# alexkreimer/libviso

Hardware: AMD Instinct MI355X
Metric: stereo_frames_per_sec_1241x376_matcher (higher is better)
Workload: dtype u16; 1 GPU; configs[1]: synthetic 1241x376 stereo pairs, 2000 features/image, SAD matcher only (pack + 3 match_desc/frame + sort)

## Files before the change

libviso_amd/csrc/match_union8.hip:

```cpp
#include "common.h"
#include "match_dev.h"
#include <stddef.h>
#include <stdlib.h>

#define MU_THREADS 256
#define MU_WAVES 4
#define MU_QPB 64
#define MU_G 8
#define MU_UCAP 448
#define MU_PAD 32
#ifndef MU_NP
#define MU_NP 2
#endif
#ifndef MU_RNP
#define MU_RNP 2
#endif
#define MU_S8ROWS 176
#define MU_KPCAP 512
#define MU_NBY 64

template <int CTRL>
__device__ __forceinline__ uint32_t mu_dpp(uint32_t v) {
    return (uint32_t)__builtin_amdgcn_update_dpp(0, (int)v, CTRL, 0xf, 0xf, false);
}

template <int CTRL>
__device__ __forceinline__ uint32_t mu_bcast(uint32_t v) {
    return (uint32_t)__builtin_amdgcn_update_dpp(0, (int)v, CTRL, 0xf, 0xf, true);
}

__device__ __forceinline__ float mu_fmin(float a, float b) { float r; asm("v_min_f32_e32 %0, %1, %2" : "=v"(r) : "v"(a), "v"(b)); return r; }
__device__ __forceinline__ float mu_fmax(float a, float b) { float r; asm("v_max_f32_e32 %0, %1, %2" : "=v"(r) : "v"(a), "v"(b)); return r; }

__device__ __forceinline__ uint32_t mu_l1_bits(float qx, float qy, float2 t) {
    const float dx = qx - t.x, dy = qy - t.y;
    float d;
    asm("v_add_f32_e64 %0, |%1|, |%2|" : "=v"(d) : "v"(dx), "v"(dy));
    return __float_as_uint(d);
}

struct MuTrack { uint32_t m1, m2, m3; };

__device__ __forceinline__ uint32_t mu_med3(uint32_t a, uint32_t b, uint32_t c) {
    uint32_t r;
    asm("v_med3_u32 %0, %1, %2, %3" : "=v"(r) : "v"(a), "v"(b), "v"(c));
    return r;
}

__device__ __forceinline__ void mu_update(MuTrack& t, uint32_t key) {
    t.m3 = mu_med3(t.m2, t.m3, key);
    t.m2 = mu_med3(t.m1, t.m2, key);
    t.m1 = min(t.m1, key);
}

__device__ __forceinline__ void mu_merge(MuTrack& a, const MuTrack& b) {
    const uint32_t c3 = min(min(a.m3, b.m3), min(max(a.m2, b.m1), max(a.m1, b.m2)));
    const uint32_t c2 = min(max(a.m1, b.m1), min(a.m2, b.m2));
    a.m1 = min(a.m1, b.m1);
    a.m2 = c2;
    a.m3 = c3;
}

__device__ __forceinline__ int mu_ybucket(float y, float y0, float scale) {
    const float f = (y - y0) * scale;
    int b;
    asm("v_cvt_i32_f32_e32 %0, %1" : "=v"(b) : "v"(f));
    return min(max(b, 0), MU_NBY - 1);
}

__device__ __forceinline__ int mu_r8s() {
    const int* kp = (const int*)__builtin_amdgcn_kernarg_segment_ptr();
    asm volatile("" : "+s"(kp));
    return kp[offsetof(BatchMatchArgs, r8s) / sizeof(int)];
}

__device__ __forceinline__ constexpr int mu_qlane(int k) { return (k & 3) + 32 * (k >> 2); }

#ifndef MU_CLK
#define MU_CLK(I) do {} while (0)
#endif
#ifndef MU_KERNEL_SIG
#define MU_KERNEL_SIG __global__ __attribute__((amdgpu_waves_per_eu(7, 8))) __launch_bounds__(MU_THREADS) void match_union8_kernel(BatchMatchArgs a)
#define MU_BLOCK blockIdx.x
#endif
MU_KERNEL_SIG {
    __shared__ __attribute__((aligned(16))) uint32_t s_ul[MU_WAVES][MU_UCAP + MU_PAD];
    __shared__ __attribute__((aligned(16))) uint32_t s_qrow[MU_WAVES][MU_G][32];
    __shared__ uint8_t s_s8[MU_WAVES][MU_G][MU_S8ROWS];
    __shared__ float2 s_ykp[MU_KPCAP];
    __shared__ uint16_t s_ypos[MU_KPCAP];
    __shared__ int s_ys[MU_NBY + 1];
    __shared__ float s_xr[2];
    int prob, qblk;
    {
        const int b = MU_BLOCK;
        const int xcd = b & 7, slot = b >> 3;
        const int g = slot / a.bpp;
        prob = ((g / a.gc) * a.gs + a.gf + g % a.gc) * 8 + xcd;
        qblk = slot % a.bpp;
        if (prob >= a.n_probs) return;
    }
    MU_CLK(0);
    const MatchProblem P = a.probs[prob];
    if ((*P.q.bad | *P.t.bad) != 0) return;
    const int n1 = *P.q.n, n2 = *P.t.n;
    const int q0 = qblk * MU_QPB;
    if (q0 >= n1) return;
    const int q1 = min(q0 + MU_QPB, n1);
    const MatchParamsDev& mp = a.mp[P.pidx];
    if (mp.epi != 0) return;
    const int wave = __builtin_amdgcn_readfirstlane(threadIdx.x >> 6), lane = threadIdx.x & 63;
    if (wave == 0) {
        const bool live = q0 + lane < q1;
        const float qx = live ? P.q.skp[q0 + lane].x : __builtin_nanf("");
        const float mn = viso_wave_fext<false>(qx), mx = viso_wave_fext<true>(qx);
        if (lane == 0) { s_xr[0] = mn; s_xr[1] = mx; }
    }
    if (threadIdx.x <= MU_NBY) s_ys[threadIdx.x] = 0;
    __syncthreads();
    int lo = 0, W = 0;
    {
        const float xa = s_xr[0], xb = s_xr[1];
        const float r = mp.radius;
        if (n2 > 0 && xa == xa && r >= 0.f) {
            const float slack = (fabsf(xa) + fabsf(xb) + fabsf(r)) * 1e-6f + 1e-6f;
            const float x0 = P.t.xinfo[0], scale = P.t.xinfo[1];
            lo = P.t.bstart[bucket_of(xa - r - slack, x0, scale)];
            W = P.t.bstart[bucket_of(xb + r + slack, x0, scale) + 1] - lo;
        }
    }
    lo = __builtin_amdgcn_readfirstlane(lo);
    W = __builtin_amdgcn_readfirstlane(W);
    const int wcap = min(W, MU_KPCAP);
    const int wpad = (wcap + 127) & ~127;
    float ty0 = P.t.xinfo[2];
    float yscale = 0.f;
    {
        const float ty1 = P.t.xinfo[3];
        if (ty1 > ty0) yscale = (float)MU_NBY / (ty1 - ty0);
        if (!(yscale > 0.f) || !(yscale < 3.0e38f)) yscale = 0.f;
    }
    ty0 = __uint_as_float(__builtin_amdgcn_readfirstlane(__float_as_uint(ty0)));
    yscale = __uint_as_float(__builtin_amdgcn_readfirstlane(__float_as_uint(yscale)));
    static_assert(MU_KPCAP <= 2 * MU_THREADS, "two window entries per thread");
    float2 e_kp[2];
    int e_b[2], e_r[2];
#pragma unroll
    for (int i = 0; i < 2; ++i) {
        const int w = threadIdx.x + i * MU_THREADS;
        e_b[i] = 0; e_r[i] = 0;
        if (w < wcap) {
            e_kp[i] = P.t.skp[lo + w];
            e_b[i] = mu_ybucket(e_kp[i].y, ty0, yscale);
            e_r[i] = atomicAdd(&s_ys[e_b[i]], 1);
        }
    }
    float2 kp0 = make_float2(0.f, 0.f);
    const bool has0 = n2 > 0;
    if (has0) kp0 = P.t.skp[P.t.rank[0]];
    kp0.x = __uint_as_float(__builtin_amdgcn_readfirstlane(__float_as_uint(kp0.x)));
    kp0.y = __uint_as_float(__builtin_amdgcn_readfirstlane(__float_as_uint(kp0.y)));
    __syncthreads();
    if (wave == 0) {
        const int h = s_ys[lane];
        const int incl = (int)viso_wave_scan((uint32_t)h);
        s_ys[lane] = incl - h;
        if (lane == VISO_WAVE - 1) s_ys[MU_NBY] = incl;
    }
    __syncthreads();
#pragma unroll
    for (int i = 0; i < 2; ++i) {
        const int w = threadIdx.x + i * MU_THREADS;
        if (w < wcap) {
            const int p = s_ys[e_b[i]] + e_r[i];
            s_ykp[p] = e_kp[i];
            s_ypos[p] = (uint16_t)w;
        } else if (w < wpad) {
            s_ykp[w] = make_float2(__builtin_nanf(""), __builtin_nanf(""));
            s_ypos[w] = 0;
        }
    }
    __syncthreads();
    const float radius = mp.radius;
    const int K = mp.K;
    typedef uint32_t u32x4 __attribute__((ext_vector_type(4)));
    typedef const __attribute__((address_space(1))) u32x4* grow_t;
    typedef const __attribute__((address_space(1))) char* gbytes_t;
    const gbytes_t wrows8 = (gbytes_t)reinterpret_cast<const char*>(P.t.rows8) + (size_t)lo * VISO_ROW8;
    const gbytes_t wrows = (gbytes_t)reinterpret_cast<const char*>(P.t.rows) + (size_t)lo * (VISO_ROW * 2);
    const gbytes_t qrows = (gbytes_t)reinterpret_cast<const char*>(P.q.rows);
    const gbytes_t qrows8 = (gbytes_t)reinterpret_cast<const char*>(P.q.rows8);
    const gbytes_t qord_b = (gbytes_t)reinterpret_cast<const char*>(P.q.qord), qskp_b = (gbytes_t)reinterpret_cast<const char*>(P.q.skp),
                   qsidx_b = (gbytes_t)reinterpret_cast<const char*>(P.q.sidx);
    uint32_t* ul = s_ul[wave];
    const int sub = lane & 7;
    const int half = lane >> 5;
    unsigned long long scored = 0;
    constexpr int ROUNDS = MU_QPB / (MU_WAVES * MU_G);
    const bool sel1 = ((lane >> 1) & 1) != 0;
    const int myq = (lane & 1) + 2 * ((lane >> 2) & 1) + (sel1 ? 4 : 0);
    const uint32_t hoff = (uint32_t)(lane & 1) << 4;
    const int msh = 31 - myq;

    const int qslot = (lane & 3) + 4 * half;
    int pli;
    float2 pq;
    int po;
#define MU_PREFETCH(R)                                                                                    \
    do {                       \
        const int base_ = wave * (MU_QPB / MU_WAVES) + (R) * MU_G;                                        \
        pli = (int)*(const __attribute__((address_space(1))) uint8_t*)(qord_b + (uint32_t)(q0 + base_ + qslot)); \
        const int j_ = q0 + pli;                                                                          \
        const int jc_ = min(j_, q1 - 1);                                                                  \
        {                                                                                                 \
            typedef float f32x2_ __attribute__((ext_vector_type(2)));                                     \
            const f32x2_ k_ = *(const __attribute__((address_space(1))) f32x2_*)(qskp_b + (uint32_t)jc_ * 8u); \
            pq = make_float2(k_.x, k_.y);                                                                 \
        }                                                                                                 \
        po = *(const __attribute__((address_space(1))) int*)(qsidx_b + (uint32_t)jc_ * 4u);             \
        po = j_ < q1 ? po : -1;                                                                           \
    } while (0)
    MU_CLK(1);
    MU_PREFETCH(0);

#pragma unroll
    for (int r = 0; r < ROUNDS; ++r) {
        const int gq_orig = __shfl(po, mu_qlane(lane >> 3)), gq_j = q0 + __shfl(pli, mu_qlane(lane >> 3));
        if (!__any(po >= 0)) { if (r + 1 < ROUNDS) MU_PREFETCH(r + 1); continue; }
        uint32_t tq = __float_as_uint(radius) + 1u;
        if (has0) {
            const float d0 = l1_kp(pq.x, pq.y, kp0);
            if (d0 <= radius) tq = __float_as_uint(d0);
        }
        if (po < 0) tq = 0u;
        tq -= 1u;
        float qx[4], qy[4];
        uint32_t thr[4];
        qx[0] = __uint_as_float(mu_bcast<0x00>(__float_as_uint(pq.x))); qy[0] = __uint_as_float(mu_bcast<0x00>(__float_as_uint(pq.y))); thr[0] = mu_bcast<0x00>(tq);
        qx[1] = __uint_as_float(mu_bcast<0x55>(__float_as_uint(pq.x))); qy[1] = __uint_as_float(mu_bcast<0x55>(__float_as_uint(pq.y))); thr[1] = mu_bcast<0x55>(tq);
        qx[2] = __uint_as_float(mu_bcast<0xAA>(__float_as_uint(pq.x))); qy[2] = __uint_as_float(mu_bcast<0xAA>(__float_as_uint(pq.y))); thr[2] = mu_bcast<0xAA>(tq);
        qx[3] = __uint_as_float(mu_bcast<0xFF>(__float_as_uint(pq.x))); qy[3] = __uint_as_float(mu_bcast<0xFF>(__float_as_uint(pq.y))); thr[3] = mu_bcast<0xFF>(tq);
        const float ymn = mu_fmin(mu_fmin(qy[0], qy[1]), mu_fmin(qy[2], qy[3]));
        const float ymx = mu_fmax(mu_fmax(qy[0], qy[1]), mu_fmax(qy[2], qy[3]));
        uint32_t qw[MU_G / 2];
        {
            const uint32_t own = (uint32_t)min(q0 + pli, q1 - 1) * (uint32_t)VISO_ROW8;
            const uint32_t l4 = (uint32_t)((lane & 31) << 2);
            qw[0] = *(const __attribute__((address_space(1))) uint32_t*)(qrows8 + (mu_bcast<0x00>(own) + l4));
            qw[1] = *(const __attribute__((address_space(1))) uint32_t*)(qrows8 + (mu_bcast<0x55>(own) + l4));
            qw[2] = *(const __attribute__((address_space(1))) uint32_t*)(qrows8 + (mu_bcast<0xAA>(own) + l4));
            qw[3] = *(const __attribute__((address_space(1))) uint32_t*)(qrows8 + (mu_bcast<0xFF>(own) + l4));
        }
        if (r + 1 < ROUNDS) MU_PREFETCH(r + 1);
        int ucnt = 0;
        uint32_t ncnt = 0, ntest = 0;
#define MU_TEST4(T)                                                                                       \
        ({                                                                                                \
            uint32_t m_ = 0;                                                                              \
            _Pragma("unroll") for (int i = 0; i < 4; ++i)                                                 \
                m_ = __builtin_amdgcn_alignbit(m_, thr[i] - mu_l1_bits(qx[i], qy[i], (T)), 31);           \
             \
                                                                             \
            const auto r_ = __builtin_amdgcn_permlane32_swap(m_, m_, false, false);                       \
            (uint32_t)((r_[0] << 4) | r_[1]);                                                             \
        })
        {
            const float ys = (fabsf(ymn) + fabsf(ymx) + fabsf(radius)) * 1e-6f + 1e-6f;
            const int h0 = s_ys[mu_ybucket(ymn - radius - ys, ty0, yscale)];
            const int h1 = s_ys[mu_ybucket(ymx + radius + ys, ty0, yscale) + 1];
            const int sc0 = min(__builtin_amdgcn_readlane(h0, 0), __builtin_amdgcn_readlane(h0, 32)) & ~63;
            const int sc1 = max(__builtin_amdgcn_readlane(h1, 0), __builtin_amdgcn_readlane(h1, 32));
            const int l31 = lane & 31;
            if (sc1 > sc0) ntest = (uint32_t)((sc1 - sc0 + 63) >> 6) * 16u;
            for (int base = sc0; base < sc1; base += 64) {
                const float2 ta = s_ykp[base + l31], tb = s_ykp[base + 32 + l31];
                const uint32_t pa = s_ypos[base + l31], pb = s_ypos[base + 32 + l31];
                const uint32_t m8a = MU_TEST4(ta), m8b = MU_TEST4(tb);
                ncnt += (uint32_t)__popc(m8a) + (uint32_t)__popc(m8b);
                const uint32_t ua = (uint32_t)__ballot(m8a != 0xffu), ub = (uint32_t)__ballot(m8b != 0xffu);
                const int ca = __popc(ua);
                if (m8a != 0xffu && half == 0) ul[min(ucnt + (int)__builtin_amdgcn_mbcnt_lo(ua, 0u), MU_UCAP - 1)] = (m8a << 24) | (pa << 7);
                if (m8b != 0xffu && half == 0) ul[min(ucnt + ca + (int)__builtin_amdgcn_mbcnt_lo(ub, 0u), MU_UCAP - 1)] = (m8b << 24) | (pb << 7);
                ucnt += ca + __popc(ub);
            }
            for (int base = wcap; base < W; base += 32) {
                const int w = base + l31;
                float2 t2 = make_float2(__builtin_nanf(""), __builtin_nanf(""));
                if (w < W) t2 = P.t.skp[lo + w];
                const uint32_t m8 = MU_TEST4(t2);
                ncnt += (uint32_t)__popc(m8);
                ntest += 8u;
                const uint32_t u = (uint32_t)__ballot(m8 != 0xffu);
                if (m8 != 0xffu && half == 0) ul[min(ucnt + (int)__builtin_amdgcn_mbcnt_lo(u, 0u), MU_UCAP - 1)] = (m8 << 24) | ((uint32_t)w << 7);
                ucnt += __popc(u);
            }
        }
#undef MU_TEST4
        const bool list_ovf = ucnt > MU_UCAP;
        const int nu = __builtin_amdgcn_readfirstlane(list_ovf ? 0 : ucnt);
        __builtin_amdgcn_wave_barrier();
        if (nu > 0 && lane < MU_PAD) ul[nu + lane] = ul[nu - 1] | 0xff000000u;
        __builtin_amdgcn_wave_barrier();
        for (int k = 0; k < MU_G / 2; ++k) s_qrow[wave][k + 4 * half][lane & 31] = qw[k];
        __builtin_amdgcn_wave_barrier();
        MuTrack tr;
        tr.m1 = 0xffffffffu; tr.m2 = 0xffffffffu; tr.m3 = 0xffffffffu;
        {
            const int npass = (nu + 7) >> 3;
            int g8 = lane;
            asm volatile("" : "+v"(g8));
            g8 >>= 3;
            u32x4 r0[MU_NP];
            uint32_t un[MU_NP];
            const uint32_t s8w = (uint32_t)(size_t)(__attribute__((address_space(3))) uint8_t*)&s_s8[wave][myq][g8];
            uint32_t s8a = s8w;
#define MU_ISSUE(SLOT, T)                                                                                  \
            do {                                                                                           \
                const uint32_t ent_ = ul[(T) * 8 + g8];                                                    \
                un[SLOT] = (uint32_t)((T) * 8 + g8) | (uint32_t)__builtin_amdgcn_sbfe((int)ent_, (uint32_t)msh, 1u); \
                const grow_t row_ = (grow_t)(wrows8 + ((ent_ & 0x00ffffffu) | (uint32_t)(sub << 4)));      \
                r0[SLOT] = row_[0];                                                                        \
            } while (0)
#define MU_SAD2(J, SLOT)                                                                                   \
            ({                                                                                             \
                const u32x4 qa_ = *reinterpret_cast<const u32x4*>(&s_qrow[wave][2 * (J)][sub * 4]);     \
                const u32x4 qb_ = *reinterpret_cast<const u32x4*>(&s_qrow[wave][2 * (J) + 1][sub * 4]); \
                uint32_t s_ = __builtin_amdgcn_sad_u8(r0[SLOT].x, qa_.x, 0u);                              \
                s_ = __builtin_amdgcn_sad_u8(r0[SLOT].y, qa_.y, s_);                                       \
                s_ = __builtin_amdgcn_sad_u8(r0[SLOT].z, qa_.z, s_);                                       \
                s_ = __builtin_amdgcn_sad_u8(r0[SLOT].w, qa_.w, s_);                                       \
                s_ = __builtin_amdgcn_sad_hi_u8(r0[SLOT].x, qb_.x, s_);                                    \
                s_ = __builtin_amdgcn_sad_hi_u8(r0[SLOT].y, qb_.y, s_);                                    \
                s_ = __builtin_amdgcn_sad_hi_u8(r0[SLOT].z, qb_.z, s_);                                    \
                s_ = __builtin_amdgcn_sad_hi_u8(r0[SLOT].w, qb_.w, s_);                                    \
                s_;                                                                                        \
            })
#define MU_X2(A, B) ({ uint32_t k_ = sel1 ? (B) : (A); const uint32_t g_ = sel1 ? (A) : (B); k_ += mu_dpp<0x4E>(g_); k_; })
#define MU_X4x2(S0, S1, S2, S3)                                                                            \
            asm("s_nop 1\n\t"                                                                              \
                "v_add_u32_dpp %0, %0, %0 row_shl:4 row_mask:0xf bank_mask:0x5\n\t"                         \
                "v_add_u32_dpp %1, %1, %1 row_shl:4 row_mask:0xf bank_mask:0x5\n\t"                         \
                "v_add_u32_dpp %0, %2, %2 row_shr:4 row_mask:0xf bank_mask:0xa\n\t"                         \
                "v_add_u32_dpp %1, %3, %3 row_shr:4 row_mask:0xf bank_mask:0xa"                              \
                : "+v"(S0), "+v"(S2) : "v"(S1), "v"(S3))
#define MU_REDUCE(SLOT, T)                                                                                \
            do {                                                                                           \
                uint32_t p0_ = MU_SAD2(0, SLOT), p1_ = MU_SAD2(1, SLOT), p2_ = MU_SAD2(2, SLOT), p3_ = MU_SAD2(3, SLOT); \
                MU_X4x2(p0_, p1_, p2_, p3_);    \
                uint32_t c_ = MU_X2(p0_, p2_);                                                             \
                c_ += mu_dpp<0xB1>(c_);               \
                const uint32_t m_ = __builtin_amdgcn_ubfe(c_, hoff, 16u);                                  \
                 \
                 \
                 \
                asm volatile("ds_write_b8 %0, %1 offset:%2" : : "v"(s8a), "v"(m_ >> 7), "n"((SLOT) * 8));    \
                mu_update(tr, (m_ << 9) | un[SLOT]);                                                       \
            } while (0)
            if (npass > 0) {
#pragma unroll
                for (int p = 0; p < MU_NP; ++p) MU_ISSUE(p, p);
            }
            int t = 0;
            for (; t + MU_NP < npass; t += MU_NP) {
#pragma unroll
                for (int p = 0; p < MU_NP; ++p) {
                    MU_REDUCE(p, t + p);
                    __builtin_amdgcn_sched_barrier(0);
                    MU_ISSUE(p, t + p + MU_NP);
                    __builtin_amdgcn_sched_barrier(0);
                }
                s8a = min(s8a + 8u * MU_NP, s8w + (MU_S8ROWS / 8 - MU_NP) * 8u);
            }
            if (npass > 0) {
#pragma unroll
                for (int p = 0; p < MU_NP; ++p)
                    if (t + p < npass) MU_REDUCE(p, t + p);
            }
#undef MU_REDUCE
#undef MU_X4x2
#undef MU_X2
#undef MU_SAD2
#undef MU_ISSUE
        }
        const int r8s = mu_r8s();
        {
            MuTrack o;
            o.m1 = mu_dpp<0x128>(tr.m1); o.m2 = mu_dpp<0x128>(tr.m2); o.m3 = mu_dpp<0x128>(tr.m3);
            mu_merge(tr, o);
            o.m1 = (uint32_t)__builtin_amdgcn_ds_swizzle((int)tr.m1, 0x401F);
            o.m2 = (uint32_t)__builtin_amdgcn_ds_swizzle((int)tr.m2, 0x401F);
            o.m3 = (uint32_t)__builtin_amdgcn_ds_swizzle((int)tr.m3, 0x401F);
            mu_merge(tr, o);
            const auto h1 = __builtin_amdgcn_permlane32_swap(tr.m1, tr.m1, false, false);
            const auto h2 = __builtin_amdgcn_permlane32_swap(tr.m2, tr.m2, false, false);
            const auto h3 = __builtin_amdgcn_permlane32_swap(tr.m3, tr.m3, false, false);
            tr.m1 = h1[0]; tr.m2 = h2[0]; tr.m3 = h3[0];
            o.m1 = h1[1]; o.m2 = h2[1]; o.m3 = h3[1];
            mu_merge(tr, o);
        }
        {
            const int k = lane >> 3;
            const int src = (lane & 0x38) | (k & 1) | ((k & 2) << 1) | ((k & 4) >> 1);
            tr.m1 = (uint32_t)__shfl((int)tr.m1, src);
            tr.m2 = (uint32_t)__shfl((int)tr.m2, src);
            tr.m3 = (uint32_t)__shfl((int)tr.m3, src);
        }
        const bool none = tr.m1 == 0xffffffffu;
        const bool has2 = tr.m2 != 0xffffffffu, has3 = tr.m3 != 0xffffffffu;
        uint32_t dA = 0, dB = 0;
        const uint32_t eA = ul[none ? 0u : (tr.m1 & 511u)], eB = ul[has2 ? (tr.m2 & 511u) : 0u];
        if (__any(!none)) {
            const grow_t ra = (grow_t)(wrows + (((eA & 0x00ffffffu) << 1) | (uint32_t)(sub << 4)));
            const grow_t rb = (grow_t)(wrows + (((eB & 0x00ffffffu) << 1) | (uint32_t)(sub << 4)));
            const grow_t rq = (grow_t)(qrows + ((uint32_t)min(gq_j, q1 - 1) * (uint32_t)(VISO_ROW * 2) + (uint32_t)(sub << 4)));
            const u32x4 a0 = ra[0], a1 = ra[8], b0 = rb[0], b1 = rb[8], x0 = rq[0], x1 = rq[8];
#define MU_SAD16(R0, R1)                                                                                   \
            ({                                                                                             \
                uint32_t s_ = __builtin_amdgcn_sad_u16((R0).x, x0.x, 0u);                                  \
                s_ = __builtin_amdgcn_sad_u16((R0).y, x0.y, s_);                                           \
                s_ = __builtin_amdgcn_sad_u16((R0).z, x0.z, s_);                                           \
                s_ = __builtin_amdgcn_sad_u16((R0).w, x0.w, s_);                                           \
                s_ = __builtin_amdgcn_sad_u16((R1).x, x1.x, s_);                                           \
                s_ = __builtin_amdgcn_sad_u16((R1).y, x1.y, s_);                                           \
                s_ = __builtin_amdgcn_sad_u16((R1).z, x1.z, s_);                                           \
                s_ = __builtin_amdgcn_sad_u16((R1).w, x1.w, s_);                                           \
                s_ += mu_dpp<0xB1>(s_);                                                      \
                s_ += mu_dpp<0x4E>(s_);                                                      \
                s_ += (uint32_t)__builtin_amdgcn_ds_swizzle((int)s_, 0x101F);                \
                s_;                                                                                        \
            })
            dA = MU_SAD16(a0, a1);
            dB = MU_SAD16(b0, b1);
#undef MU_SAD16
        }
        const bool mine = sub == 0 && gq_orig >= 0;
        uint32_t kA = none ? 0xffffffffu : ((dA << 9) | (tr.m1 & 511u)), kB = has2 ? ((dB << 9) | (tr.m2 & 511u)) : 0xffffffffu;
        bool accept = !none, irregular = false, rescue = false;
        if (!none && has2) {
            const uint32_t d1 = min(dA, dB), d2 = max(dA, dB);
            const int L3 = (int)((tr.m3 >> 9) << r8s) - VISO_ROW8_SLACK(r8s);
            if (mp.second) {
                const double lim = (double)d2 * mp.ratio;
                accept = (double)d1 < lim;
                if (has3) rescue = !(accept ? (L3 > (int)d1 && (double)d1 < (double)L3 * mp.ratio) : ((double)L3 >= lim));
            } else if (has3) {
                rescue = !(L3 > (int)d1);
            }
            if (dA == dB) { irregular = true; rescue = false; }
        } else if (!none && mp.second) {
            accept = (double)dA < 1.7976931348623157e308 * mp.ratio;
        }
        {
            asm volatile("" ::: "memory");
            unsigned long long rm = __ballot(rescue && sub == 0);
            const int g8 = lane >> 3;
            uint16_t* ml = reinterpret_cast<uint16_t*>(&s_qrow[wave][0][0]);
            uint32_t* qst = &s_qrow[wave][4][0];
            static_assert(MU_S8ROWS <= 256, "the survivor list holds every position that may survive");
            if (nu > MU_S8ROWS) {
                rm = 0;
                if (rescue) { irregular = true; rescue = false; }
            }
#define MU_UPD2(KEY) do { const uint32_t k_ = (KEY); m2 = mu_med3(m1, m2, k_); m1 = min(m1, k_); } while (0)
            while (rm) {
                const int bit = __builtin_ctzll(rm);
                rm &= rm - 1;
                const int k = bit >> 3;
                const int jq = min(__builtin_amdgcn_readlane(gq_j, bit), q1 - 1);
                const uint32_t ka = (uint32_t)__builtin_amdgcn_readlane((int)kA, bit), kb = (uint32_t)__builtin_amdgcn_readlane((int)kB, bit);
                const uint32_t pa = ka & 511u, pb = kb & 511u;
                const int d1k = (int)(min(ka, kb) >> 9);
                const double limk = (double)(max(ka, kb) >> 9) * mp.ratio;
                const bool acck = !mp.second || (double)d1k < limk;
                const uint32_t msk = 31u - (uint32_t)k;
                const int r8q = mu_r8s();
                const uint32_t qv = *(const __attribute__((address_space(1))) uint32_t*)(qrows + ((uint32_t)jq * (uint32_t)(VISO_ROW * 2) + (uint32_t)(lane << 2)));
                __builtin_amdgcn_wave_barrier();
                int nm = 0;
                for (int b = 0; b < nu; b += VISO_WAVE) {
                    const uint32_t i = (uint32_t)(b + lane);
                    bool sel = false;
                    if (i < (uint32_t)nu) {
                        const uint32_t e = ul[i];
                        const uint32_t q8 = s_s8[wave][k][i];
                        const int Lt = (int)(q8 << (7 + r8q)) - VISO_ROW8_SLACK(r8q);
                        const bool clear = q8 == 255u || (!mp.second ? Lt > d1k : (acck ? (Lt > d1k && (double)d1k < (double)Lt * mp.ratio) : ((double)Lt >= limk)));
                        sel = ((e >> msk) & 1u) == 0 && !clear && i != pa && i != pb;
                        if (sel) s_s8[wave][k][i] = 255;
                    }
                    const unsigned long long bal = __ballot(sel);
                    if (sel) ml[nm + mbcnt(bal)] = (uint16_t)i;
                    nm += __popcll(bal);
                }
                __builtin_amdgcn_wave_barrier();
                qst[lane] = qv;
                if (nm > 0 && lane < 8 * MU_RNP) ml[nm + lane] = ml[nm - 1];
                __builtin_amdgcn_wave_barrier();
                uint32_t m1 = 0xffffffffu, m2 = 0xffffffffu;
                if (nm > 0) {
                    for (int t = 0; t * 8 < nm; t += MU_RNP) {
                        uint32_t pos[MU_RNP];
                        u32x4 a0[MU_RNP], a1[MU_RNP];
#pragma unroll
                        for (int p = 0; p < MU_RNP; ++p) {
                            pos[p] = ml[(t + p) * 8 + g8];
                            const grow_t ra = (grow_t)(wrows + (((ul[pos[p]] & 0x00ffffffu) << 1) | (uint32_t)(sub << 4)));
                            a0[p] = ra[0]; a1[p] = ra[8];
                        }
#pragma unroll
                        for (int p = 0; p < MU_RNP; ++p) {
                            int o_ = sub * 4;
                            asm volatile("" : "+v"(o_));
                            const u32x4 x0_ = *reinterpret_cast<const u32x4*>(&qst[o_]);
                            uint32_t sa = __builtin_amdgcn_sad_u16(a0[p].x, x0_.x, 0u);
                            sa = __builtin_amdgcn_sad_u16(a0[p].y, x0_.y, sa);
                            sa = __builtin_amdgcn_sad_u16(a0[p].z, x0_.z, sa);
                            sa = __builtin_amdgcn_sad_u16(a0[p].w, x0_.w, sa);
                            const u32x4 x1_ = *reinterpret_cast<const u32x4*>(&qst[o_ + 32]);
                            sa = __builtin_amdgcn_sad_u16(a1[p].x, x1_.x, sa);
                            sa = __builtin_amdgcn_sad_u16(a1[p].y, x1_.y, sa);
                            sa = __builtin_amdgcn_sad_u16(a1[p].z, x1_.z, sa);
                            sa = __builtin_amdgcn_sad_u16(a1[p].w, x1_.w, sa);
                            sa += mu_dpp<0xB1>(sa);
                            sa += mu_dpp<0x4E>(sa);
                            sa += (uint32_t)__builtin_amdgcn_ds_swizzle((int)sa, 0x101F);
                            MU_UPD2(((t + p) * 8 + g8 < nm && sub == 0) ? ((sa << 9) | pos[p]) : 0xffffffffu);
                        }
                    }
#define MU_MRG2(O1, O2) do { const uint32_t o1_ = (O1), o2_ = (O2); m2 = min(max(m1, o1_), min(m2, o2_)); m1 = min(m1, o1_); } while (0)
                    MU_MRG2(mu_dpp<0x128>(m1), mu_dpp<0x128>(m2));
                    MU_MRG2((uint32_t)__builtin_amdgcn_ds_swizzle((int)m1, 0x401F), (uint32_t)__builtin_amdgcn_ds_swizzle((int)m2, 0x401F));
                    {
                        const auto h1 = __builtin_amdgcn_permlane32_swap(m1, m1, false, false);
                        const auto h2 = __builtin_amdgcn_permlane32_swap(m2, m2, false, false);
                        m1 = h1[0]; m2 = h2[0];
                        MU_MRG2(h1[1], h2[1]);
                    }
#undef MU_MRG2
                }
                bool again = false;
                if (g8 == k) {
                    MU_UPD2(kA);
                    MU_UPD2(kB);
                    kA = m1; kB = m2;
                    accept = !mp.second || (double)(m1 >> 9) < (double)(m2 >> 9) * mp.ratio;
                    again = accept && !acck;
                }
                if (__any(again)) rm |= 1ull << bit;
            }
#undef MU_UPD2
            if (rescue && (kA >> 9) == (kB >> 9)) irregular = true;
        }
        const uint32_t kwin = min(kA, kB);
        const uint32_t d1 = kwin >> 9;
        const uint32_t ewin = ul[none ? 0u : (kwin & 511u)];
        const bool slow = nu > K || __any(mine && irregular);
        int my_cnt = 0;
        if (slow) {
            for (int b = 0; b < nu; b += VISO_WAVE) {
                const uint32_t e = (b + lane) < nu ? ul[b + lane] : 0xffffffffu;
#pragma unroll
                for (int k = 0; k < MU_G; ++k) {
                    const int c = __popcll(__ballot(((e >> (31 - k)) & 1u) == 0));
                    if ((lane >> 3) == k) my_cnt += c;
                }
            }
        } else if (!list_ovf && half == 0) {
            scored += ntest - ncnt;
        }
        if (mine) {
            if (list_ovf || my_cnt > K || irregular) {
                P.ovf[atomicAdd(P.ovf_cnt, 1)] = make_int2(prob, gq_j);
            } else {
                int idx = -1;
                if (accept) {
                    const int w = (int)((ewin & 0x00ffffffu) >> 7);
                    idx = P.t.sidx[lo + w];
                }
                P.res[gq_orig] = make_int2(idx, none ? -1 : (int)d1);
                if (slow) scored += (unsigned long long)my_cnt;
            }
        }
        MU_CLK(2 + r);
    }
    scored = viso_wave_sum63(scored);
    if (lane == 63 && scored) atomicAdd(P.scored, scored);
}

#ifndef MU_NO_LAUNCHER
int launch_match_union8_temporal(hipStream_t s, const BatchMatchArgs& a, long long blocks) {
    size_t pad = 0;
#ifdef VISO_DEBUG_VARIANTS
    { static const int p = [] { const char* e = getenv("VISO_EXP_U8_LDS_PAD"); return e ? atoi(e) : 0; }(); if (p > 0 && p < 32768) pad = (size_t)p; }
#endif
    hipLaunchKernelGGL(match_union8_kernel, dim3((unsigned)blocks), dim3(MU_THREADS), pad, s, a);
    hipError_t e = hipGetLastError();
    if (e != hipSuccess) { viso_set_error("match_union8_kernel launch: %s", hipGetErrorString(e)); return VISO_ERR_HIP; }
    return VISO_OK;
}
#endif
```

Before: 509,900 frames/s.

## Recompute coarse 8-bit SAD in rescue path instead of caching per-candidate bytes

Removes the per-candidate ds_write_b8 of the coarse SAD from the main matching loop and the s_s8 shared buffer. The rescue path now builds a member list and recomputes the coarse 8-bit SAD on demand from the row data, tracking already-handled candidates in a per-wave bitmask. This lightens the hot inner loop and shared-memory footprint, at the cost of extra global loads and SAD work whenever a rescue happens. It also drops the old cap on list size for rescue.

```diff
diff --git a/libviso_amd/csrc/match_union8.hip b/libviso_amd/csrc/match_union8.hip
--- a/libviso_amd/csrc/match_union8.hip
+++ b/libviso_amd/csrc/match_union8.hip
@@ -15,7 +15,6 @@
 #ifndef MU_RNP
 #define MU_RNP 2
 #endif
-#define MU_S8ROWS 176
 #define MU_KPCAP 512
 #define MU_NBY 64
 
@@ -86,7 +85,8 @@
 MU_KERNEL_SIG {
     __shared__ __attribute__((aligned(16))) uint32_t s_ul[MU_WAVES][MU_UCAP + MU_PAD];
     __shared__ __attribute__((aligned(16))) uint32_t s_qrow[MU_WAVES][MU_G][32];
-    __shared__ uint8_t s_s8[MU_WAVES][MU_G][MU_S8ROWS];
+    __shared__ __attribute__((aligned(16))) uint32_t s_rq[MU_WAVES][64];
+    __shared__ uint32_t s_done[MU_WAVES][(MU_UCAP + 31) / 32];
     __shared__ float2 s_ykp[MU_KPCAP];
     __shared__ uint16_t s_ypos[MU_KPCAP];
     __shared__ int s_ys[MU_NBY + 1];
@@ -312,8 +312,6 @@
             g8 >>= 3;
             u32x4 r0[MU_NP];
             uint32_t un[MU_NP];
-            const uint32_t s8w = (uint32_t)(size_t)(__attribute__((address_space(3))) uint8_t*)&s_s8[wave][myq][g8];
-            uint32_t s8a = s8w;
 #define MU_ISSUE(SLOT, T)                                                                                  \
             do {                                                                                           \
                 const uint32_t ent_ = ul[(T) * 8 + g8];                                                    \
@@ -350,10 +348,6 @@
                 uint32_t c_ = MU_X2(p0_, p2_);                                                             \
                 c_ += mu_dpp<0xB1>(c_);               \
                 const uint32_t m_ = __builtin_amdgcn_ubfe(c_, hoff, 16u);                                  \
-                 \
-                 \
-                 \
-                asm volatile("ds_write_b8 %0, %1 offset:%2" : : "v"(s8a), "v"(m_ >> 7), "n"((SLOT) * 8));    \
                 mu_update(tr, (m_ << 9) | un[SLOT]);                                                       \
             } while (0)
             if (npass > 0) {
@@ -369,7 +363,6 @@
                     MU_ISSUE(p, t + p + MU_NP);
                     __builtin_amdgcn_sched_barrier(0);
                 }
-                s8a = min(s8a + 8u * MU_NP, s8w + (MU_S8ROWS / 8 - MU_NP) * 8u);
             }
             if (npass > 0) {
 #pragma unroll
@@ -451,16 +444,13 @@
             accept = (double)dA < 1.7976931348623157e308 * mp.ratio;
         }
         {
-            asm volatile("" ::: "memory");
             unsigned long long rm = __ballot(rescue && sub == 0);
             const int g8 = lane >> 3;
             uint16_t* ml = reinterpret_cast<uint16_t*>(&s_qrow[wave][0][0]);
-            uint32_t* qst = &s_qrow[wave][4][0];
-            static_assert(MU_S8ROWS <= 256, "the survivor list holds every position that may survive");
-            if (nu > MU_S8ROWS) {
-                rm = 0;
-                if (rescue) { irregular = true; rescue = false; }
-            }
+            uint32_t* qst = s_rq[wave];
+            uint32_t* done = s_done[wave];
+            static_assert((MU_UCAP + 8 * MU_RNP) * 2 <= MU_G * 32 * 4, "the member list holds every position of the round's list");
+            bool redo = false;
 #define MU_UPD2(KEY) do { const uint32_t k_ = (KEY); m2 = mu_med3(m1, m2, k_); m1 = min(m1, k_); } while (0)
             while (rm) {
                 const int bit = __builtin_ctzll(rm);
@@ -468,29 +458,60 @@
                 const int k = bit >> 3;
                 const int jq = min(__builtin_amdgcn_readlane(gq_j, bit), q1 - 1);
                 const uint32_t ka = (uint32_t)__builtin_amdgcn_readlane((int)kA, bit), kb = (uint32_t)__builtin_amdgcn_readlane((int)kB, bit);
-                const uint32_t pa = ka & 511u, pb = kb & 511u;
                 const int d1k = (int)(min(ka, kb) >> 9);
                 const double limk = (double)(max(ka, kb) >> 9) * mp.ratio;
                 const bool acck = !mp.second || (double)d1k < limk;
                 const uint32_t msk = 31u - (uint32_t)k;
                 const int r8q = mu_r8s();
+                const u32x4 qp = *(grow_t)(qrows8 + ((uint32_t)jq * (uint32_t)VISO_ROW8 + (uint32_t)(sub << 4)));
                 const uint32_t qv = *(const __attribute__((address_space(1))) uint32_t*)(qrows + ((uint32_t)jq * (uint32_t)(VISO_ROW * 2) + (uint32_t)(lane << 2)));
+                if (!redo) {
+                    if (lane < (MU_UCAP + 31) / 32) done[lane] = 0u;
+                    __builtin_amdgcn_wave_barrier();
+                    if (lane < 2) { const uint32_t p_ = (lane ? kb : ka) & 511u; atomicOr(&done[p_ >> 5], 1u << (p_ & 31u)); }
+                }
+                __builtin_amdgcn_wave_barrier();
+                int nc = 0;
+                for (int b = 0; b < nu; b += VISO_WAVE) {
+                    const uint32_t i = (uint32_t)(b + lane);
+                    bool mem = false;
+                    if (i < (uint32_t)nu) mem = ((ul[i] >> msk) & 1u) == 0 && ((done[i >> 5] >> (i & 31u)) & 1u) == 0;
+                    const unsigned long long bal = __ballot(mem);
+                    if (mem) ml[nc + mbcnt(bal)] = (uint16_t)i;
+                    nc += __popcll(bal);
+                }
+                __builtin_amdgcn_wave_barrier();
+                if (nc > 0 && lane < 8 * MU_RNP) ml[nc + lane] = ml[nc - 1];
                 __builtin_amdgcn_wave_barrier();
                 int nm = 0;
-                for (int b = 0; b < nu; b += VISO_WAVE) {
-                    const uint32_t i = (uint32_t)(b + lane);
-                    bool sel = false;
-                    if (i < (uint32_t)nu) {
-                        const uint32_t e = ul[i];
-                        const uint32_t q8 = s_s8[wave][k][i];
-                        const int Lt = (int)(q8 << (7 + r8q)) - VISO_ROW8_SLACK(r8q);
-                        const bool clear = q8 == 255u || (!mp.second ? Lt > d1k : (acck ? (Lt > d1k && (double)d1k < (double)Lt * mp.ratio) : ((double)Lt >= limk)));
-                        sel = ((e >> msk) & 1u) == 0 && !clear && i != pa && i != pb;
-                        if (sel) s_s8[wave][k][i] = 255;
+                for (int t = 0; t * 8 < nc; t += MU_RNP) {
+                    uint32_t pos[MU_RNP];
+                    u32x4 rw[MU_RNP];
+#pragma unroll
+                    for (int p = 0; p < MU_RNP; ++p) {
+                        pos[p] = ml[(t + p) * 8 + g8];
+                        rw[p] = *(grow_t)(wrows8 + ((ul[pos[p]] & 0x00ffffffu) | (uint32_t)(sub << 4)));
                     }
-                    const unsigned long long bal = __ballot(sel);
-                    if (sel) ml[nm + mbcnt(bal)] = (uint16_t)i;
-                    nm += __popcll(bal);
+                    __builtin_amdgcn_wave_barrier();
+#pragma unroll
+                    for (int p = 0; p < MU_RNP; ++p) {
+                        uint32_t s8 = __builtin_amdgcn_sad_u8(rw[p].x, qp.x, 0u);
+                        s8 = __builtin_amdgcn_sad_u8(rw[p].y, qp.y, s8);
+                        s8 = __builtin_amdgcn_sad_u8(rw[p].z, qp.z, s8);
+                        s8 = __builtin_amdgcn_sad_u8(rw[p].w, qp.w, s8);
+                        s8 += mu_dpp<0xB1>(s8);
+                        s8 += mu_dpp<0x4E>(s8);
+                        s8 += (uint32_t)__builtin_amdgcn_ds_swizzle((int)s8, 0x101F);
+                        const int Lt = (int)(s8 << r8q) - VISO_ROW8_SLACK(r8q);
+                        const bool clear = !mp.second ? Lt > d1k : (acck ? (Lt > d1k && (double)d1k < (double)Lt * mp.ratio) : ((double)Lt >= limk));
+                        const bool sel = (t + p) * 8 + g8 < nc && !clear && sub == 0;
+                        const unsigned long long bal = __ballot(sel);
+                        if (sel) {
+                            ml[nm + mbcnt(bal)] = (uint16_t)pos[p];
+                            atomicOr(&done[pos[p] >> 5], 1u << (pos[p] & 31u));
+                        }
+                        nm += __popcll(bal);
+                    }
                 }
                 __builtin_amdgcn_wave_barrier();
                 qst[lane] = qv;
@@ -546,7 +567,8 @@
                     accept = !mp.second || (double)(m1 >> 9) < (double)(m2 >> 9) * mp.ratio;
                     again = accept && !acck;
                 }
-                if (__any(again)) rm |= 1ull << bit;
+                redo = __any(again);
+                if (redo) rm |= 1ull << bit;
             }
 #undef MU_UPD2
             if (rescue && (kA >> 9) == (kB >> 9)) irregular = true;
```

Result: no change. 510,000 frames/s (median of 2 runs) (+0.0%).
